# CILAB-MA/gpudrive_lab

Hardware: AMD Instinct MI355X
Metric: agent-steps/sec at 1024 worlds x 64 agents; achieved HBM GB/s on obs kernel (higher is better)
Workload: dtype f32

## Files before the change

gpudrive_lab_amd/csrc/map_obs_rank.hip:

```cpp
#include <hip/hip_runtime.h>

#include <algorithm>
#include <type_traits>

#include "engine.hpp"
#include "gd_math.hpp"
#include "rank_cand.hpp"
#include "rank_heap.hpp"

namespace gd {

namespace {

constexpr int K = GD_MAP_OBS_K;
constexpr int CAP = GD_RANK_CAP;
constexpr int NCP = GD_RANK_NCP;
constexpr int SPL = GD_RANK_SPL;
constexpr int KT = GD_RANK_KT;
constexpr int TILE = 32;
constexpr int CAP_LONG = GD_RANK_CAP_LONG;
template <int CAP_T>
struct RankGeo {
    static constexpr bool LONG = CAP_T > CAP;
    static constexpr int NG = CAP_T / 64;
    static constexpr int NMAX = CAP_T - 8;
    static constexpr int NB = CAP_T;
    static constexpr int NLIN = CAP_T * 3 / 5;
    static constexpr int TSH = LONG ? 6 : 5;
    static constexpr int RSH = LONG ? 4 : 5;
    static constexpr int KTN = LONG ? GD_RANK_KT_LONG : GD_RANK_KT;
};
constexpr int NB = RankGeo<CAP>::NB;
static_assert(K + (NCP - 1) * TILE >= CAP && K + (NCP - 1) * 64 >= CAP_LONG, "a checkpoint slot for every tile of candidates");
static_assert(CAP % 64 == 0 && NB % 128 == 0 && CAP < 2047 && CAP_LONG % 640 == 0 && CAP_LONG < 4095, "geometry; less + 1 fits 11 / 12 bits");
static_assert(SPL >= K + 31 && SPL <= CAP && KT >= CAP / 16 + 1, "every slot the finish looks up; an entry per 16 slots + the last");
constexpr int RK_FAR = 1 << 30;
constexpr int RK_TIES = 1 << 30;

__device__ __forceinline__ void wave_sync() {
    __builtin_amdgcn_fence(__ATOMIC_RELEASE, "wavefront");
    __builtin_amdgcn_wave_barrier();
    __builtin_amdgcn_fence(__ATOMIC_ACQUIRE, "wavefront");
}

__device__ __forceinline__ int wave_incl_scan(int v) {
    v += __builtin_amdgcn_update_dpp(0, v, 0x111, 0xf, 0xf, false);
    v += __builtin_amdgcn_update_dpp(0, v, 0x112, 0xf, 0xf, false);
    v += __builtin_amdgcn_update_dpp(0, v, 0x114, 0xf, 0xf, false);
    v += __builtin_amdgcn_update_dpp(0, v, 0x118, 0xf, 0xf, false);
    v += __builtin_amdgcn_update_dpp(0, v, 0x142, 0xa, 0xf, false);
    v += __builtin_amdgcn_update_dpp(0, v, 0x143, 0xc, 0xf, false);
    return v;
}

#define GD_DPP_SELF(v, ctrl, rows) __builtin_amdgcn_update_dpp((v), (v), (ctrl), (rows), 0xf, false)
__device__ __forceinline__ int wave_max(int v) {
    v = max(v, GD_DPP_SELF(v, 0x111, 0xf));
    v = max(v, GD_DPP_SELF(v, 0x112, 0xf));
    v = max(v, GD_DPP_SELF(v, 0x114, 0xf));
    v = max(v, GD_DPP_SELF(v, 0x118, 0xf));
    v = max(v, GD_DPP_SELF(v, 0x142, 0xa));
    v = max(v, GD_DPP_SELF(v, 0x143, 0xc));
    return __builtin_amdgcn_readlane(v, 63);
}
__device__ __forceinline__ float wave_max_nonneg(float f) { return __int_as_float(wave_max(__float_as_int(f))); }
__device__ __forceinline__ float wave_min_nonneg(float f) { return __int_as_float(~wave_max(~__float_as_int(f))); }
__device__ __forceinline__ int wave_sum(int v) { return __builtin_amdgcn_readlane(wave_incl_scan(v), 63); }
__device__ __forceinline__ int bits_below_lane(unsigned long long b) {
    return (int)__builtin_amdgcn_mbcnt_hi((unsigned int)(b >> 32), __builtin_amdgcn_mbcnt_lo((unsigned int)b, 0u));
}

#ifndef GD_NT_FINISH_LOAD
#define GD_NT_FINISH_LOAD 1
#endif
#ifndef GD_NT_REPLAY_LOAD
#define GD_NT_REPLAY_LOAD 1
#endif
typedef unsigned int u4v __attribute__((ext_vector_type(4)));
typedef unsigned int u2v __attribute__((ext_vector_type(2)));
template <typename T>
__device__ __forceinline__ T stream_load(const T *p) { return __builtin_nontemporal_load(p); }
template <typename T>
__device__ __forceinline__ void stream_store(T v, T *p) { __builtin_nontemporal_store(v, p); }
__device__ __forceinline__ uint4 stream_load(const uint4 *p) {
    const u4v v = __builtin_nontemporal_load(reinterpret_cast<const u4v *>(p));
    return make_uint4(v.x, v.y, v.z, v.w);
}
__device__ __forceinline__ void stream_store(uint4 v, uint4 *p) {
    u4v t; t.x = v.x; t.y = v.y; t.z = v.z; t.w = v.w;
    __builtin_nontemporal_store(t, reinterpret_cast<u4v *>(p));
}
__device__ __forceinline__ uint2 stream_load(const uint2 *p) {
    const u2v v = __builtin_nontemporal_load(reinterpret_cast<const u2v *>(p));
    return make_uint2(v.x, v.y);
}
__device__ __forceinline__ void stream_store(uint2 v, uint2 *p) {
    u2v t; t.x = v.x; t.y = v.y;
    __builtin_nontemporal_store(t, reinterpret_cast<u2v *>(p));
}

__device__ __forceinline__ int audited(const DevSim &d, int idx, int size) {
    if ((unsigned int)idx < (unsigned int)size) return idx;
    atomicAdd(&d.rk_hist[GD_RANK_AUDIT], 1);
    return idx < 0 ? 0 : size - 1;
}

__device__ __forceinline__ bool rank_lt(unsigned int a, unsigned int b, unsigned int tm = 31u) { return (a | tm) < b; }

template <int A_T>
__global__ __launch_bounds__(256) void k_knn_scan(DevSim d) {
    if (d.gate_any && *d.any_reset == 0) return;
    constexpr int HALVES = A_T / 64;
    const int w = blockIdx.x / HALVES, a0 = (blockIdx.x % HALVES) * 64;
    const int tid = threadIdx.x, wave = tid >> 6, lane = tid & 63;
    const int n = d.shape[w * 2 + 0];
    if (a0 >= n) return;
    const int a = a0 + lane;
    const bool live = a < n;
    const size_t i = (size_t)w * A_T + a;
    const size_t WA = (size_t)d.W * A_T;
    const int r0 = d.road_off[w];
    const int R = d.road_off[w + 1] - r0;

    __shared__ unsigned short s_first[NCP][64];
    __shared__ float s_thr[NCP][64];
    __shared__ int s_ncp[64];
    __shared__ unsigned int s_needy[2];
    __shared__ float4 s_hdr[64];
    __shared__ float s_bx[64], s_by[64], s_bm[64];
    __shared__ unsigned int s_hist[4][256];

    float ex = 0.f, ey = 0.f;
    if (live) { ex = d.px[i]; ey = d.py[i]; }
    unsigned long long ranked = 0ull;
    int list_base = 0;
    if (wave == 0) {
        int ncp = 0;
        float4 h0 = make_float4(0.f, 0.f, __int_as_float(0), 0.f), h1 = h0;
        if (live) { h0 = d.cp_hdr[i]; h1 = d.cp_hdr[WA + i]; }
        s_hdr[lane] = h0;
        wave_sync();
        if (live) {
            const float4 bb = d.road_bbox[w];
            const float ddx = fmaxf(fmaxf(bb.x - ex, ex - bb.z), 0.f), ddy = fmaxf(fmaxf(bb.y - ey, ey - bb.w), 0.f);
            const float far = d.p.observationRadius * 1.01f + 1.f;
            int state = 1, reason = -1;
            if (R >= K && ddx * ddx + ddy * ddy > far * far) {
                state = RK_FAR;
                d.sel_hdr[i * 2] = make_float4(ex, ey, d.qw[i], d.qz[i]);
                d.sel_hdr[i * 2 + 1] = make_float4(__int_as_float(0), __int_as_float(r0), 0.f, 0.f);
                d.cp_hdr[i] = make_float4(ex, ey, __int_as_float(0), 0.f);
            } else {
                const int n0 = __float_as_int(h0.z), n1 = __float_as_int(h1.z);
                const float m0 = n0 > 0 ? sqrtf((ex - h0.x) * (ex - h0.x) + (ey - h0.y) * (ey - h0.y)) : __builtin_inff();
                const float m1 = n1 > 0 ? sqrtf((ex - h1.x) * (ex - h1.x) + (ey - h1.y) * (ey - h1.y)) : __builtin_inff();
                int set = m1 < m0 ? 1 : 0;
                float move = set ? m1 : m0;
                int n_cp = set ? n1 : n0;
                size_t src = i;
                if (move > 6.f) {
                    float best = move;
                    int donor = -1;
                    for (int j = 0; j < 64; j++) {
                        const float4 hj = s_hdr[j];
                        const float dj = __float_as_int(hj.z) > 0 ? sqrtf((ex - hj.x) * (ex - hj.x) + (ey - hj.y) * (ey - hj.y)) : __builtin_inff();
                        if (dj < best) { best = dj; donor = j; }
                    }
                    if (donor >= 0) {
                        move = best;
                        set = 0;
                        n_cp = __float_as_int(s_hdr[donor].z);
                        src = (size_t)w * A_T + a0 + donor;
                    }
                }
                const bool eligible = R >= K && R >= d.rk_min_roads && R <= d.rk_max_roads;
                const int grp = (int)(i / 32);
                const bool bypass = eligible && d.rk_streak[grp] >= 3 && ((d.rk_hist[513] + grp) & 63) != 0;
                const float iw = d.qw[i], iz = d.qz[i];
                const float z2 = iz * iz;
                const float det = (1.f - 2.f * z2) * (1.f - 2.f * z2) + 4.f * z2 * (iw * iw);
                const float margin = 1.00001f / fminf(det, 1.f);
                if (!eligible || bypass) {
                    state = 0;
                    ncp = 0;
                    reason = bypass ? -5 : -2;
                    d.rk_fallback[i / 32] = 1;
                } else if (n_cp <= 0 || move > 6.f) {
                    ncp = -1;
                    s_bx[lane] = ex; s_by[lane] = ey; s_bm[lane] = margin;
                } else {
                    ncp = n_cp;
                    const unsigned short *cr = d.cp_road + ((size_t)set * WA + src) * NCP;
                    const float *ct = d.cp_T + ((size_t)set * WA + src) * NCP;
                    float t = 1.f;
                    unsigned int fmax = 0u;
                    for (int q = 0; q < ncp; q++) {
                        t = ct[q];
                        const float reach = sqrtf(t) * 1.0001f + move * 1.0001f + 1e-3f;
                        float thr = reach * reach * 1.0001f * margin;
                        if (!(thr >= 0.f)) thr = __builtin_inff();
                        fmax = rank_cand::running_max(fmax, cr[q]);
                        s_first[q][lane] = (unsigned short)fmax;
                        s_thr[q][lane] = thr;
                    }
                    d.rk_tl[i] = t;
                }
            }
            d.rk_n[i] = state;
            d.rk_ticket[i] = reason;
            if (state == RK_FAR) ncp = 0;
        }
        s_ncp[lane] = ncp;
        {
            const unsigned long long nd = __ballot(ncp < 0);
            if (lane == 0) { s_needy[0] = (unsigned int)nd; s_needy[1] = (unsigned int)(nd >> 32); }
        }
        if (ncp < 0) ncp = 1;
        ranked = __ballot(ncp > 0);
        if (ranked != 0ull && lane == 0) list_base = atomicAdd(&d.rk_hist[528 + (blockIdx.x & 7)], __popcll(ranked));
    }
    __syncthreads();
    {
        const unsigned long long needy = (unsigned long long)s_needy[0] | (unsigned long long)s_needy[1] << 32;
        if (needy != 0ull) {
            constexpr int BASE = (127 - 2) << 4;
            unsigned int *hist = s_hist[wave];
            int turn = 0;
            for (unsigned long long rest = needy; rest != 0ull; rest &= rest - 1ull, turn++) {
                if ((turn & 3) != wave) continue;
                const int al = __ffsll((long long)rest) - 1;
                const float bx = s_bx[al], by = s_by[al], mg = s_bm[al];
#pragma unroll
                for (int k = 0; k < 4; k++) hist[k * 64 + lane] = 0u;
                if (lane == 0) { s_first[0][al] = (unsigned short)((K / 32) * 32); s_thr[0][al] = __builtin_inff(); }
                const float ratio = exp2f(log2f(fmaxf((float)R / 256.f, 1.f)) / (float)(NCP - 2));
                float pf = 256.f, tlast = __builtin_inff();
                int pq = 256, q = 1;
                float2 nxt = lane < R ? d.road_xy[r0 + lane] : make_float2(0.f, 0.f);
                for (int rb = 0; rb < R; rb += 64) {
                    const float2 xy = nxt;
                    if (rb + 64 + lane < R) nxt = d.road_xy[r0 + rb + 64 + lane];
                    if (rb + lane < R) {
                        const float dx = xy.x - bx, dy = xy.y - by;
                        const float d2 = __builtin_fmaf(dx, dx, dy * dy);
                        atomicAdd(&hist[min(255, max(0, (int)(__float_as_uint(d2) >> 19) - BASE))], 1u);
                    }
                    if (rb + 64 == pq && q < NCP && pq < R) {
                        wave_sync();
                        const uint4 h = reinterpret_cast<const uint4 *>(hist)[lane];
                        const int own = (int)(h.x + h.y + h.z + h.w);
                        const int incl = wave_incl_scan(own), excl = incl - own;
                        int jb = 0, before = excl;
                        if (before + (int)h.x < K) { before += (int)h.x; jb = 1;
                            if (before + (int)h.y < K) { before += (int)h.y; jb = 2;
                                if (before + (int)h.z < K) { jb = 3; } } }
                        const unsigned long long cross = __ballot(excl < K && incl >= K);
                        const int Lc = __ffsll((long long)cross) - 1;
                        const int bucket = 4 * Lc + __builtin_amdgcn_readlane(jb, Lc);
                        const float T = bucket >= 255 ? __builtin_inff() : __uint_as_float((unsigned int)(bucket + 1 + BASE) << 19);
                        if (lane == 0) {
                            const float reach = sqrtf(T) * 1.0001f + 1e-3f;
                            float thr = reach * reach * 1.0001f * mg * 1.001f;
                            if (!(thr >= 0.f)) thr = __builtin_inff();
                            s_first[q][al] = (unsigned short)min(pq, 65535);
                            s_thr[q][al] = thr;
                        }
                        tlast = T;
                        q++;
                        pf *= ratio;
                        pq = max(pq + 64, ((int)pf + 63) & ~63);
                    }
                }
                if (lane == 0) {
                    s_ncp[al] = q;
                    d.rk_tl[(size_t)w * A_T + a0 + al] = tlast < 1e30f ? tlast : 1.f;
                }
            }
            __syncthreads();
        }
    }
    const int ncp = s_ncp[lane];
    if (__syncthreads_or(ncp > 0 ? 1 : 0) == 0) return;
    {
        uint2 *rows = d.rk_cp + ((size_t)w * A_T + a0) * NCP;
        for (int e = tid; e < 64 * NCP; e += 256) {
            const int ag = e / NCP, q = e - ag * NCP;
            const int n_ag = s_ncp[ag];
            if (n_ag > 0)
                rows[e] = q < n_ag ? make_uint2((unsigned int)s_first[q][ag], __float_as_uint(s_thr[q][ag]))
                                   : make_uint2(rank_cand::NO_CP, __float_as_uint(__builtin_inff()));
        }
    }
    if (wave == 0 && ranked != 0ull) {
        list_base = __builtin_amdgcn_readfirstlane(list_base);
        if (ncp > 0)
            d.rk_list[(size_t)(blockIdx.x & 7) * WA + audited(d, list_base + __popcll(ranked & ((1ull << lane) - 1ull)), (int)WA)] = (int)i;
    }
}

template <int CAP_T>
struct RankLds {
    union {
        struct {
            float ckey[CAP_T];
            unsigned short cidx[CAP_T];
        } c;
        struct {
            float skey[CAP_T];
            unsigned short spos[CAP_T];
        } s;
        unsigned short spc[CAP_T];
    };
    unsigned int cnt2[RankGeo<CAP_T>::NB / 2];
};
static_assert(sizeof(RankLds<CAP>) <= 10240 && sizeof(RankLds<CAP_LONG>) <= 20480, "sixteen / eight waves per CU");
constexpr int LSTN = (GD_MAX_ROAD_ENTITIES + GD_LIN_BLK - 1) / GD_LIN_BLK + 15;
constexpr int LSTN4 = (LSTN + 3) & ~3;
static_assert(LSTN4 <= 1024 && NCP < 64 && rank_cand::CHUNK % GD_LIN_BLK == 0 && 64 % GD_LIN_BLK == 0, "block and count share 16 bits; a block inside one chunk; whole blocks per pass");
constexpr size_t CAND_TABLES = LSTN4 * sizeof(unsigned short) + (NCP + 1) * sizeof(float);
static_assert(CAND_TABLES <= sizeof(RankLds<CAP>::cnt2) && CAND_TABLES <= sizeof(RankLds<CAP_LONG>::cnt2), "the tables fit the idle counters of both instantiations");

struct RankIn {
    int i, state, r0, R, b0, li;
    float ex, ey, iw, iz, t_last;
    unsigned int cfirst;
    float cthr;
};
template <typename T>
__device__ __forceinline__ T uniform_load(const T *p) {
    return *reinterpret_cast<const __attribute__((address_space(4))) T *>(reinterpret_cast<uintptr_t>(p));
}
template <int A_T>
__device__ __forceinline__ RankIn rank_fetch(const DevSim &d, const int *list, int li, int count, int lane) {
    RankIn in;
    in.li = li;
    in.i = li < count ? uniform_load(list + li) : 0;
    in.state = li < count ? uniform_load(d.rk_n + in.i) : 0;
    const int w = in.i / A_T;
    in.r0 = uniform_load(d.road_off + w);
    in.R = uniform_load(d.road_off + w + 1) - in.r0;
    in.ex = uniform_load(d.px + in.i); in.ey = uniform_load(d.py + in.i);
    in.iw = uniform_load(d.qw + in.i); in.iz = -uniform_load(d.qz + in.i);
    in.t_last = uniform_load(d.rk_tl + in.i);
    in.b0 = uniform_load(d.blk_off + w);
    uint2 cp = make_uint2(rank_cand::NO_CP, __float_as_uint(__builtin_inff()));
    if (in.state == 1 && lane < NCP) cp = stream_load(d.rk_cp + (size_t)in.i * NCP + (unsigned int)lane);
    in.cfirst = cp.x;
    in.cthr = __uint_as_float(cp.y);
    return in;
}

#ifdef GD_CLOCKS
struct PhaseClock {
    unsigned int prev, sum[8];
    __device__ __forceinline__ void mark(int n) {
        const unsigned int t = (unsigned int)__builtin_amdgcn_s_memtime();
        sum[n] += t - prev;
        prev = t;
    }
};
#define GD_PHASE(n) clk.mark(n)
#else
struct PhaseClock {};
#define GD_PHASE(n)
#endif
template <int A_T, int CAP_T>
__device__ __forceinline__ void rank_agent(const DevSim &d, const RankIn &in, int lane, RankLds<CAP_T> &L, PhaseClock &clk, int next_entry,
                                           int count, const int *list, RankIn &nxt) {
    using G = RankGeo<CAP_T>;
    constexpr int NB = G::NB, NLIN = G::NLIN, NMAX = G::NMAX;
    constexpr unsigned int TM = (1u << G::RSH) - 1u;
    if (__builtin_amdgcn_readfirstlane(in.state) != 1) {
        nxt = rank_fetch<A_T>(d, list, next_entry, count, lane);
        return;
    }
    auto uni = [](int v) -> int { return __builtin_amdgcn_readfirstlane(v); };
    auto unif = [](float v) -> float { return __int_as_float(__builtin_amdgcn_readfirstlane(__float_as_int(v))); };
    const int i = uni(in.i), r0 = uni(in.r0), R = uni(in.R);
    const int group = i / 32;
    constexpr int NG = G::NG;

    const float ex = unif(in.ex), ey = unif(in.ey), iw = unif(in.iw), iz = unif(in.iz);
    unsigned short *const lst = reinterpret_cast<unsigned short *>(L.cnt2);
    float *const tthr = reinterpret_cast<float *>(L.cnt2) + LSTN4 / 2;
    const unsigned int cfirst = in.cfirst;
    if (lane < NCP) tthr[lane + 1] = in.cthr;
    if (lane == 63) tthr[0] = __builtin_inff();
    const float creach = rank_cand::block_reach(in.cthr);
    const int nblk = (R + GD_LIN_BLK - 1) / GD_LIN_BLK;
    const float4 *blk = d.road_blk + uni(in.b0);
    int nsv = 0;
    constexpr int CU = 4;
#pragma clang loop unroll(disable)
    for (int b0 = 0; b0 < nblk; b0 += 64 * CU) {
        float4 c[CU];
#pragma unroll
        for (int u = 0; u < CU; u++) c[u] = blk[(unsigned int)min(b0 + u * 64 + lane, nblk - 1)];
#pragma unroll
        for (int u = 0; u < CU; u++) {
            const int bb = b0 + u * 64;
            if (bb < nblk) {
                const int b = bb + lane;
                const unsigned int base = (unsigned int)rank_cand::chunk_base_of_block(b, GD_LIN_BLK);
                const unsigned int base_lo = (unsigned int)rank_cand::chunk_base_of_block(bb, GD_LIN_BLK);
                const unsigned int base_hi = (unsigned int)rank_cand::chunk_base_of_block(min(bb + 63, nblk - 1), GD_LIN_BLK);
                const int nlo = __popcll(__ballot(cfirst <= base_lo)), nhi = __popcll(__ballot(cfirst <= base_hi));
                int cnt = nlo;
                for (int q = nlo; q < nhi; q++) cnt += (unsigned int)__builtin_amdgcn_readlane((int)cfirst, q) <= base ? 1 : 0;
                const float reach = __int_as_float(__builtin_amdgcn_ds_bpermute(((cnt - 1) & 63) << 2, __float_as_int(creach)));
                const bool sv = b < nblk && rank_cand::block_survives(b, GD_LIN_BLK, K, c[u].x, c[u].y, c[u].z, ex, ey, reach);
                const unsigned long long m = __ballot(sv);
                if (sv) lst[audited(d, nsv + bits_below_lane(m), LSTN4)] = (unsigned short)(b | cnt << 10);
                nsv += __popcll(m);
            }
        }
    }
    wave_sync();
    int nin = 0;
    {
        constexpr int BPP = 64 / GD_LIN_BLK, PB = 2;
        const int np = (nsv + BPP - 1) / BPP;
        const int sub = lane / GD_LIN_BLK, o = lane % GD_LIN_BLK;
        const float2 *rxy = d.road_xy + r0;
        struct Batch { int r[PB]; float thr[PB]; float2 xy[PB]; };
        auto issue = [&](Batch &bt, int p0) {
#pragma unroll
            for (int u = 0; u < PB; u++) {
                const int e = (p0 + u) * BPP + sub;
                const unsigned int ent = lst[min(e, LSTN4 - 1)];
                const bool on = e < nsv;
                const int r = on ? (int)(ent & 1023u) * GD_LIN_BLK + o : R;
                bt.r[u] = r;
                bt.thr[u] = tthr[on ? min((int)(ent >> 10), NCP) : 0];
                bt.xy[u] = rxy[(unsigned int)min(r, R - 1)];
            }
        };
        auto take = [&](const Batch &bt) {
#pragma unroll
            for (int u = 0; u < PB; u++) {
                const bool cand = rank_cand::is_candidate(bt.r[u], K, R, bt.xy[u].x, bt.xy[u].y, ex, ey, bt.thr[u]);
                const float key = ego_dist2(ex, ey, iw, iz, bt.xy[u].x, bt.xy[u].y);
                const unsigned long long m = __ballot(cand);
                const int pos = nin + bits_below_lane(m);
                if (cand && pos < CAP_T) {
                    L.c.cidx[pos] = (unsigned short)bt.r[u];
                    L.c.ckey[pos] = key;
                }
                nin += __popcll(m);
            }
        };
        Batch ba, bb;
        issue(ba, 0);
#pragma clang loop unroll(disable)
        for (int p0 = 0; p0 < np; p0 += 2 * PB) {
            issue(bb, p0 + PB);
            take(ba);
            if (p0 + PB >= np) break;
            issue(ba, p0 + 2 * PB);
            take(bb);
        }
    }
    wave_sync();
    nxt = rank_fetch<A_T>(d, list, next_entry, count, lane);
    {
        const int total = nin;
        if (total > NMAX) {
            if (lane == 0) {
                bool passed_on = false;
                if (!G::LONG && total <= RankGeo<CAP_LONG>::NMAX) {
                    const int slot = atomicAdd(&d.rk_hist[GD_RH_LONG], 1);
                    if (slot < d.rk_nlong) {
                        d.rk_longlist[slot] = i;
                        passed_on = true;
                    }
                }
                if (!passed_on) {
                    d.rk_n[i] = 0;
                    d.rk_ticket[i] = -3;
                    d.rk_fallback[group] = 1;
                }
            }
            return;
        }
    }
#ifdef GD_CLOCKS
    clk.sum[7] += (unsigned int)((nsv + 3) / 4) << 8;
#endif
    const int bin = 255 - min(255, (nin - K) / 5);
    int ticket = 0;
    if (lane == 0) ticket = bin << 20 | atomicAdd(&d.rk_hist[bin], 1);
    GD_PHASE(1);
    if (GD_DIAG_IS(d.rk_dbg, 1)) return;
    if (lane <= (nin - K) >> G::TSH) {
        const int road = (int)L.c.cidx[K - 1 + (lane << G::TSH)];
        d.cp_road[(size_t)i * NCP + lane] = (unsigned short)(lane ? min(65535, (road + 1 + 31) & ~31) : (K / 32) * 32);
    }
    constexpr int GQ = 5;
    static_assert(NG % GQ == 0, "whole groups");
    const float kmax = d.radius_key_max;
    int ci[NG];
    float key[NG];
    const float t_last = unif(in.t_last);
    float split = (t_last > 0.f && t_last < 1e30f) ? t_last * 1.5f : 1.f;
    int nle = 0, nlow = 0;
    float kmax_seen = 0.f, kmin_seen = __builtin_inff();
#pragma unroll
    for (int g0 = 0; g0 < NG; g0 += GQ) {
#pragma unroll
        for (int u = 0; u < GQ; u++) { ci[g0 + u] = 0; key[g0 + u] = 0.f; }
        if (g0 * 64 < nin) {
            int v[GQ];
            float kv[GQ];
#pragma unroll
            for (int u = 0; u < GQ; u++) {
                v[u] = (int)L.c.cidx[(g0 + u) * 64 + lane];
                kv[u] = L.c.ckey[(g0 + u) * 64 + lane];
            }
            static_assert(GQ == 5, "operand list");
            asm volatile("" : "+v"(v[0]), "+v"(v[1]), "+v"(v[2]), "+v"(v[3]), "+v"(v[4]), "+v"(kv[0]), "+v"(kv[1]), "+v"(kv[2]), "+v"(kv[3]), "+v"(kv[4]));
#pragma unroll
            for (int u = 0; u < GQ; u++) {
                const int g = g0 + u;
                const bool on = g * 64 + lane < nin;
                ci[g] = on ? v[u] : 0;
                key[g] = on ? kv[u] : 0.f;
                nle += ((on & (key[g] <= kmax)) ? 1 : 0) + ((on & (key[g] < split)) ? 1 << 16 : 0);
                kmax_seen = fmaxf(kmax_seen, key[g]);
                kmin_seen = fminf(kmin_seen, on ? key[g] : __builtin_inff());
            }
        }
    }
    wave_sync();
    nle = wave_sum(nle);
    kmax_seen = wave_max_nonneg(kmax_seen);
    kmin_seen = wave_min_nonneg(kmin_seen);
    nlow = nle >> 16;
    nle &= 0xffff;
    GD_PHASE(2);
    if (GD_DIAG_IS(d.rk_dbg, 2)) return;

    for (int b = lane; b < NB / 2; b += 64) L.cnt2[b] = 0u;
    wave_sync();
    const bool jumped = nlow * 4 < nin || nlow == nin;
    const float lin_lo = jumped ? kmin_seen : 0.f;
    const int nlin = jumped ? NB : NLIN;
    const float lin_scale = jumped ? (float)NB / fmaxf(kmax_seen - kmin_seen, 1e-30f) : (float)NLIN / split;
    if (jumped) split = __builtin_inff();
    const unsigned int split_bits = __float_as_uint(split);
    const float log_scale = (float)(NB - NLIN) / (float)(max(__float_as_uint(kmax_seen), split_bits + 1u) - split_bits + 1u);
    auto bucket_of = [&](float k) -> int {
        if (k < split) return min(nlin - 1, max(0, (int)((k - lin_lo) * lin_scale)));
        return NLIN + min(NB - NLIN - 1, (int)((float)(__float_as_uint(k) - split_bits) * log_scale));
    };
#pragma unroll
    for (int g = 0; g < NG; g++) {
        if (g * 64 < nin) {
            const int b = bucket_of(key[g]);
            ci[g] |= b << 16;
            if (g * 64 + lane < nin) atomicAdd(&L.cnt2[b >> 1], 1u << ((b & 1) * 16));
        }
    }
    wave_sync();
    {
        constexpr int WPB = NB / 64 / 2;
        static_assert(WPB * 128 == NB, "whole counter words per lane");
        unsigned int own[WPB];
        int sum = 0;
#pragma unroll
        for (int k = 0; k < WPB; k++) { own[k] = L.cnt2[lane * WPB + k]; sum += (int)(own[k] & 0xffffu) + (int)(own[k] >> 16); }
        int run = wave_incl_scan(sum) - sum;
#pragma unroll
        for (int k = 0; k < WPB; k++) {
            const int lo = run, hi = run + (int)(own[k] & 0xffffu);
            run = hi + (int)(own[k] >> 16);
            L.cnt2[lane * WPB + k] = (unsigned int)lo | (unsigned int)hi << 16;
        }
    }
    wave_sync();
    GD_PHASE(3);
    if (GD_DIAG_IS(d.rk_dbg, 3)) return;
#pragma unroll
    for (int g0 = 0; g0 < NG; g0 += GQ) {
        if (g0 * 64 < nin) {
            int sl[GQ];
#pragma unroll
            for (int u = 0; u < GQ; u++) {
                const int b = ci[g0 + u] >> 16, sh = (b & 1) * 16;
                const unsigned int one = (g0 + u) * 64 + lane < nin ? 1u << sh : 0u;
                sl[u] = (int)((atomicAdd(&L.cnt2[b >> 1], one) >> sh) & 0xffffu);
            }
#pragma unroll
            for (int u = 0; u < GQ; u++) {
                if ((g0 + u) * 64 + lane < nin) {
                    L.s.skey[sl[u]] = key[g0 + u];
                    L.s.spos[sl[u]] = (unsigned short)((g0 + u) * 64 + lane);
                }
            }
        }
    }
    wave_sync();
    GD_PHASE(4);
    if (GD_DIAG_IS(d.rk_dbg, 4)) return;
    const unsigned short *cur16 = reinterpret_cast<const unsigned short *>(L.cnt2);
    unsigned int eqmask = 0u;
    float *const kt_row = G::LONG ? d.rk_kt_long + (size_t)uni(in.li) * G::KTN : d.rk_kt + (size_t)i * G::KTN;
    if (lane == 0) kt_row[(nin + 15) >> 4] = kmax_seen;
    constexpr int U = 4, M = 6, STEP = 4;
    const int lim = nin;
    if (lane < 8) L.s.skey[nin + lane] = __builtin_inff();
    wave_sync();
#pragma unroll
    for (int g0 = 0; g0 < NG; g0 += U) {
        if (g0 * 64 >= nin) break;
        int s0[U], s1[U], less[U], eq[U], longest = 0;
#pragma unroll
        for (int u = 0; u < U; u++) {
            const int b = ci[g0 + u] >> 16;
            s0[u] = b ? (int)cur16[b - 1] : 0;
            s1[u] = (g0 + u) * 64 + lane < nin ? (int)cur16[b] : s0[u];
        }
#pragma unroll
        for (int u = 0; u < U; u++) {
            float mk[M];
            static_assert(M <= 8, "end markers");
#pragma unroll
            for (int k = 0; k < M; k++) mk[k] = L.s.skey[s0[u] + k];
            less[u] = s0[u];
            eq[u] = 0;
            longest = max(longest, s1[u] - s0[u]);
#pragma unroll
            for (int k = 0; k < M; k++) {
                less[u] += mk[k] < key[g0 + u] ? 1 : 0;
                eq[u] += mk[k] == key[g0 + u] ? 1 : 0;
            }
        }
        longest = wave_max(longest);
        if (GD_DIAG_IS(d.rk_dbg, 7)) longest = 0;
#ifdef GD_DIAG
        if (lane == 0 && d.rk_dbg == 9) atomicMax(&d.rk_hist[514], longest);
#endif
        for (int j = M; j < longest; j += STEP) {
            float mkk[U][STEP];
#pragma unroll
            for (int u = 0; u < U; u++)
#pragma unroll
                for (int k = 0; k < STEP; k++) mkk[u][k] = L.s.skey[min(s0[u] + j + k, lim)];
#pragma unroll
            for (int u = 0; u < U; u++)
#pragma unroll
                for (int k = 0; k < STEP; k++) {
                    less[u] += mkk[u][k] < key[g0 + u] ? 1 : 0;
                    eq[u] += mkk[u][k] == key[g0 + u] ? 1 : 0;
                }
        }
#pragma unroll
        for (int u = 0; u < U; u++) {
            const bool on = (g0 + u) * 64 + lane < nin;
            eqmask |= ((eq[u] > 1) & on) ? 1u << (g0 + u) : 0u;
            ci[g0 + u] = (ci[g0 + u] & 0xffff) | ((less[u] + 1) << (16 + G::RSH));
            const int j = (less[u] + 15) >> 4;
            if (on && (j << 4) < less[u] + eq[u]) kt_row[j] = key[g0 + u];
        }
    }
    int too_many_ties = 0;
    const bool has_tie = __ballot(eqmask != 0u) != 0ull;
    if (has_tie) {
#pragma clang loop unroll(disable)
        for (int g = 0; g * 64 < nin; g++) {
            if (__ballot((eqmask >> g) & 1u) == 0ull) continue;
            int cg = 0;
#pragma unroll
            for (int k = 0; k < NG; k++) cg = k == g ? ci[k] : cg;
            int tie = 0;
            if ((eqmask >> g) & 1u) {
                const int less_g = (int)((unsigned int)cg >> (16 + G::RSH)) - 1, p = g * 64 + lane;
                int lo = 0, hi = NB - 1;
#pragma clang loop unroll(disable)
                while (lo < hi) {
                    const int mid = (lo + hi) >> 1;
                    if ((int)cur16[mid] > less_g) hi = mid; else lo = mid + 1;
                }
                const int b = lo;
                const int first = b ? (int)cur16[b - 1] : 0, end = (int)cur16[b];
                float kg = 0.f;
                for (int m = first; m < end; m++) kg = (int)L.s.spos[m] == p ? L.s.skey[m] : kg;
                for (int m = first; m < end; m++) tie += (L.s.skey[m] == kg ? 1 : 0) & ((int)L.s.spos[m] < p ? 1 : 0);
            }
            too_many_ties |= tie > (int)TM ? 1 : 0;
#pragma unroll
            for (int k = 0; k < NG; k++) ci[k] |= k == g ? (tie & (int)TM) << 16 : 0;
        }
    }
    wave_sync();
    GD_PHASE(5);
    if (GD_DIAG_IS(d.rk_dbg, 5)) return;
    if (__ballot(too_many_ties != 0) != 0ull) {
        if (lane == 0) {
            d.rk_n[i] = 0;
            d.rk_ticket[i] = ticket | RK_TIES;
            d.rk_fallback[group] = 1;
        }
        return;
    }
    unsigned short *const E_row = G::LONG ? d.rk_E_long + (size_t)uni(in.li) * CAP_LONG : d.rk_E + (size_t)i * CAP;
    const unsigned int ulane = (unsigned int)lane;
#pragma unroll
    for (int g = 0; g < NG; g++) {
        if (g * 64 < nin) {
            if (g * 64 + lane < nin) {
                const unsigned int e = (unsigned int)ci[g] >> 16;
                stream_store((unsigned short)e, E_row + (g * 64u + ulane));
                const int slot = (int)(e >> G::RSH) - 1 + (int)(e & TM);
                if (slot < SPL) L.spc[slot] = (unsigned short)(ci[g] & 0xffff);
            }
        }
    }
    wave_sync();
    {
        static_assert(SPL == 256, "four slots per lane");
        const uint2 v = reinterpret_cast<const uint2 *>(L.spc)[lane];
        stream_store(v, reinterpret_cast<uint2 *>(d.rk_spc + (size_t)i * SPL) + ulane);
    }
    if (lane == 0) {
        d.rk_n[i] = nin | (nle << 16) | (has_tie ? 1 << 28 : 0) | (G::LONG ? 1 << 29 : 0);
        if (G::LONG) d.rk_longslot[i] = uni(in.li);
        d.rk_ticket[i] = ticket;
    }
    GD_PHASE(6);
}

template <int A_T, int CAP_T>
__global__ __launch_bounds__(64, CAP_T > CAP ? 2 : 4) void k_knn_rank(DevSim d) {
    if (d.gate_any && *d.any_reset == 0) return;
    __shared__ RankLds<CAP_T> L;
    constexpr bool LONG = RankGeo<CAP_T>::LONG;
    const int stride = LONG ? (int)gridDim.x : (int)(gridDim.x >> 3);
    const int xcd = blockIdx.x & 7;
    const int count = LONG ? min(uniform_load(d.rk_hist + GD_RH_LONG), d.rk_nlong) : uniform_load(d.rk_hist + 528 + xcd);
    const int *list = LONG ? d.rk_longlist : d.rk_list + (size_t)xcd * d.W * A_T;
    int t = LONG ? (int)blockIdx.x : (int)(blockIdx.x >> 3);
    RankIn cur = rank_fetch<A_T>(d, list, t, count, threadIdx.x);
    PhaseClock clk;
#ifdef GD_CLOCKS
    for (int k = 0; k < 8; k++) clk.sum[k] = 0u;
    clk.prev = (unsigned int)__builtin_amdgcn_s_memtime();
#endif
    for (; t < count; t += stride) {
        RankIn nxt;
        GD_PHASE(0);
        int lane_v = threadIdx.x;
        asm volatile("" : "+v"(lane_v));
        rank_agent<A_T, CAP_T>(d, cur, lane_v, L, clk, t + stride, count, list, nxt);
        wave_sync();
        cur = nxt;
    }
#ifdef GD_CLOCKS
    if (threadIdx.x == 0)
        for (int k = 0; k < 8; k++) atomicAdd(reinterpret_cast<unsigned int *>(&d.rk_hist[516 + k]), clk.sum[k] >> 8);
#endif
}

#ifndef GD_RANK_AWR
// ... 411 lines not shown
```

gpudrive_lab_amd/csrc/rank_cand.hpp:

```cpp
#pragma once

#include <cmath>

#if defined(__HIPCC__)
#define GD_RC_FN __host__ __device__ __forceinline__
#else
#define GD_RC_FN inline
#endif

namespace gd {
namespace rank_cand {

constexpr int CHUNK = 32;
constexpr unsigned int NO_CP = 0xffffffffu;

GD_RC_FN unsigned int f32_bits(float f) { return __builtin_bit_cast(unsigned int, f); }

GD_RC_FN bool road_passes(float x, float y, float ex, float ey, float thr) {
    const float dx = x - ex, dy = y - ey;
    const float d2 = __builtin_fmaf(dx, dx, dy * dy);
    return (f32_bits(d2 - thr) >> 31) != 0u;
}
GD_RC_FN bool is_candidate(int r, int K, int R, float x, float y, float ex, float ey, float thr) {
    return r < R && (r < K || road_passes(x, y, ex, ey, thr));
}

GD_RC_FN int cp_in_force(const unsigned int *first, int ncp, int base) {
    int q = -1;
    while (q + 1 < ncp && first[q + 1] <= (unsigned int)base) q++;
    return q;
}
GD_RC_FN unsigned int running_max(unsigned int run, unsigned int first) { return first > run ? first : run; }
GD_RC_FN int cp_count(const unsigned int *first_max, int n, int base) {
    int c = 0;
    for (int q = 0; q < n; q++) c += first_max[q] <= (unsigned int)base ? 1 : 0;
    return c;
}
GD_RC_FN int chunk_base_of_block(int b, int blk) { return (b * blk) & ~(CHUNK - 1); }

GD_RC_FN float block_reach(float thr) { return sqrtf(thr) * 1.00001f; }
GD_RC_FN bool block_survives(int b, int blk, int K, float cx, float cy, float rad, float ex, float ey, float reach) {
    const float dx = cx - ex, dy = cy - ey, rr = reach + rad;
    return b * blk < K || !(dx * dx + dy * dy > rr * rr * 1.00001f);
}

}
}
```

Before: 65.83 million.

## Precompute per-chunk checkpoint table in LDS and add unguarded fast candidate pass

Before scanning road blocks, the kernel builds a per-chunk table in LDS that holds the checkpoint count and reach, using an atomicMax scatter followed by a wave prefix-max. This replaces the per-block ballot and readlane loop over checkpoints. The candidate gather gets a fast path that reads packed list entries as words with bitfield extracts and skips the CAP bounds check while there is room, with a guarded tail loop handling the rest. It also drops the audited store in favour of an overflow counter. In exchange it adds LDS setup and barriers per agent and reuses the candidate-key region as scratch space.

```diff
diff --git a/gpudrive_lab_amd/csrc/map_obs_rank.hip b/gpudrive_lab_amd/csrc/map_obs_rank.hip
--- a/gpudrive_lab_amd/csrc/map_obs_rank.hip
+++ b/gpudrive_lab_amd/csrc/map_obs_rank.hip
@@ -53,6 +53,16 @@
     return v;
 }
 
+__device__ __forceinline__ int wave_incl_max_nonneg(int v) {
+    v = max(v, __builtin_amdgcn_update_dpp(0, v, 0x111, 0xf, 0xf, false));
+    v = max(v, __builtin_amdgcn_update_dpp(0, v, 0x112, 0xf, 0xf, false));
+    v = max(v, __builtin_amdgcn_update_dpp(0, v, 0x114, 0xf, 0xf, false));
+    v = max(v, __builtin_amdgcn_update_dpp(0, v, 0x118, 0xf, 0xf, false));
+    v = max(v, __builtin_amdgcn_update_dpp(0, v, 0x142, 0xa, 0xf, false));
+    v = max(v, __builtin_amdgcn_update_dpp(0, v, 0x143, 0xc, 0xf, false));
+    return v;
+}
+
 #define GD_DPP_SELF(v, ctrl, rows) __builtin_amdgcn_update_dpp((v), (v), (ctrl), (rows), 0xf, false)
 __device__ __forceinline__ int wave_max(int v) {
     v = max(v, GD_DPP_SELF(v, 0x111, 0xf));
@@ -66,6 +76,7 @@
 __device__ __forceinline__ float wave_max_nonneg(float f) { return __int_as_float(wave_max(__float_as_int(f))); }
 __device__ __forceinline__ float wave_min_nonneg(float f) { return __int_as_float(~wave_max(~__float_as_int(f))); }
 __device__ __forceinline__ int wave_sum(int v) { return __builtin_amdgcn_readlane(wave_incl_scan(v), 63); }
+__device__ __forceinline__ unsigned long long wave_ballot(bool p) { return __builtin_amdgcn_ballot_w64(p); }
 __device__ __forceinline__ int bits_below_lane(unsigned long long b) {
     return (int)__builtin_amdgcn_mbcnt_hi((unsigned int)(b >> 32), __builtin_amdgcn_mbcnt_lo((unsigned int)b, 0u));
 }
@@ -319,6 +330,8 @@
 static_assert(LSTN4 <= 1024 && NCP < 64 && rank_cand::CHUNK % GD_LIN_BLK == 0 && 64 % GD_LIN_BLK == 0, "block and count share 16 bits; a block inside one chunk; whole blocks per pass");
 constexpr size_t CAND_TABLES = LSTN4 * sizeof(unsigned short) + (NCP + 1) * sizeof(float);
 static_assert(CAND_TABLES <= sizeof(RankLds<CAP>::cnt2) && CAND_TABLES <= sizeof(RankLds<CAP_LONG>::cnt2), "the tables fit the idle counters of both instantiations");
+constexpr int CP_EPL = ((GD_MAX_ROAD_ENTITIES + rank_cand::CHUNK - 1) / rank_cand::CHUNK + 63) / 64;
+static_assert(64 * CP_EPL * (sizeof(unsigned int) + sizeof(uint2)) <= sizeof(float) * CAP, "the chunk table fits the candidate keys of both instantiations");
 
 struct RankIn {
     int i, state, r0, R, b0, li;
@@ -388,30 +401,61 @@
     if (lane == 63) tthr[0] = __builtin_inff();
     const float creach = rank_cand::block_reach(in.cthr);
     const int nblk = (R + GD_LIN_BLK - 1) / GD_LIN_BLK;
+    const int nch = rank_cand::chunks_of(R), epl = (nch + 63) >> 6;
+    unsigned int *const tmax = reinterpret_cast<unsigned int *>(L.c.ckey);
+    uint2 *const tcp = reinterpret_cast<uint2 *>(L.c.ckey + 64 * CP_EPL);
+#pragma unroll
+    for (int u = 0; u < CP_EPL; u++)
+        if (u < epl) tmax[u * 64 + lane] = 0u;
+    wave_sync();
+    if (lane < NCP && rank_cand::cp_table_takes(cfirst, nch)) atomicMax(&tmax[rank_cand::cp_table_chunk(cfirst)], rank_cand::cp_table_entry(lane));
+    wave_sync();
+    {
+        int own[CP_EPL], run = 0;
+#pragma unroll
+        for (int u = 0; u < CP_EPL; u++) own[u] = u < epl ? (int)tmax[lane * epl + u] : 0;
+#pragma unroll
+        for (int u = 0; u < CP_EPL; u++) { run = max(run, own[u]); own[u] = run; }
+        const int before = __builtin_amdgcn_ds_bpermute(((lane - 1) & 63) << 2, wave_incl_max_nonneg(run));
+#pragma unroll
+        for (int u = 0; u < CP_EPL; u++)
+            if (u < epl) {
+                const int cnt = lane ? max(own[u], before) : own[u];
+                const int reach = __builtin_amdgcn_ds_bpermute(((cnt - 1) & 63) << 2, __float_as_int(creach));
+                tcp[lane * epl + u] = make_uint2((unsigned int)cnt, (unsigned int)reach);
+            }
+    }
+    wave_sync();
     const float4 *blk = d.road_blk + uni(in.b0);
     int nsv = 0;
     constexpr int CU = 4;
 #pragma clang loop unroll(disable)
     for (int b0 = 0; b0 < nblk; b0 += 64 * CU) {
         float4 c[CU];
-#pragma unroll
-        for (int u = 0; u < CU; u++) c[u] = blk[(unsigned int)min(b0 + u * 64 + lane, nblk - 1)];
+        uint2 cp[CU];
+#pragma unroll
+        for (int u = 0; u < CU; u++) {
+            const int bc = min(b0 + u * 64 + lane, nblk - 1);
+            c[u] = blk[(unsigned int)bc];
+            cp[u] = tcp[rank_cand::chunk_base_of_block(bc, GD_LIN_BLK) / rank_cand::CHUNK];
+        }
+        static_assert(CU == 4, "operand list");
+        asm volatile("" : "+v"(c[0].x), "+v"(c[0].y), "+v"(c[0].z), "+v"(c[1].x), "+v"(c[1].y), "+v"(c[1].z), "+v"(c[2].x), "+v"(c[2].y), "+v"(c[2].z),
+                     "+v"(c[3].x), "+v"(c[3].y), "+v"(c[3].z));
 #pragma unroll
         for (int u = 0; u < CU; u++) {
             const int bb = b0 + u * 64;
             if (bb < nblk) {
                 const int b = bb + lane;
-                const unsigned int base = (unsigned int)rank_cand::chunk_base_of_block(b, GD_LIN_BLK);
-                const unsigned int base_lo = (unsigned int)rank_cand::chunk_base_of_block(bb, GD_LIN_BLK);
-                const unsigned int base_hi = (unsigned int)rank_cand::chunk_base_of_block(min(bb + 63, nblk - 1), GD_LIN_BLK);
-                const int nlo = __popcll(__ballot(cfirst <= base_lo)), nhi = __popcll(__ballot(cfirst <= base_hi));
-                int cnt = nlo;
-                for (int q = nlo; q < nhi; q++) cnt += (unsigned int)__builtin_amdgcn_readlane((int)cfirst, q) <= base ? 1 : 0;
-                const float reach = __int_as_float(__builtin_amdgcn_ds_bpermute(((cnt - 1) & 63) << 2, __float_as_int(creach)));
-                const bool sv = b < nblk && rank_cand::block_survives(b, GD_LIN_BLK, K, c[u].x, c[u].y, c[u].z, ex, ey, reach);
-                const unsigned long long m = __ballot(sv);
-                if (sv) lst[audited(d, nsv + bits_below_lane(m), LSTN4)] = (unsigned short)(b | cnt << 10);
-                nsv += __popcll(m);
+                const bool sv = b < nblk && rank_cand::block_survives(b, GD_LIN_BLK, K, c[u].x, c[u].y, c[u].z, ex, ey, __uint_as_float(cp[u].y));
+                const unsigned long long m = wave_ballot(sv);
+                const int upto = nsv + __popcll(m);
+                if (upto <= LSTN4) {
+                    if (sv) lst[nsv + bits_below_lane(m)] = (unsigned short)((unsigned int)b | cp[u].x << 10);
+                    nsv = upto;
+                } else if (lane == 0) {
+                    atomicAdd(&d.rk_hist[GD_RANK_AUDIT], 1);
+                }
             }
         }
     }
@@ -419,45 +463,85 @@
     int nin = 0;
     {
         constexpr int BPP = 64 / GD_LIN_BLK, PB = 2;
-        const int np = (nsv + BPP - 1) / BPP;
+        const int np = (nsv + BPP - 1) / BPP, nfast = np - 1;
         const int sub = lane / GD_LIN_BLK, o = lane % GD_LIN_BLK;
         const float2 *rxy = d.road_xy + r0;
-        struct Batch { int r[PB]; float thr[PB]; float2 xy[PB]; };
-        auto issue = [&](Batch &bt, int p0) {
-#pragma unroll
-            for (int u = 0; u < PB; u++) {
-                const int e = (p0 + u) * BPP + sub;
-                const unsigned int ent = lst[min(e, LSTN4 - 1)];
-                const bool on = e < nsv;
-                const int r = on ? (int)(ent & 1023u) * GD_LIN_BLK + o : R;
-                bt.r[u] = r;
-                bt.thr[u] = tthr[on ? min((int)(ent >> 10), NCP) : 0];
-                bt.xy[u] = rxy[(unsigned int)min(r, R - 1)];
-            }
+        auto store = [&](bool cand, int r, float key, unsigned long long m, bool guard) {
+            const int pos = nin + bits_below_lane(m);
+            if (cand && (!guard || pos < CAP_T)) {
+                L.c.cidx[pos] = (unsigned short)r;
+                L.c.ckey[pos] = key;
+            }
+            nin += __popcll(m);
         };
-        auto take = [&](const Batch &bt) {
-#pragma unroll
-            for (int u = 0; u < PB; u++) {
-                const bool cand = rank_cand::is_candidate(bt.r[u], K, R, bt.xy[u].x, bt.xy[u].y, ex, ey, bt.thr[u]);
-                const float key = ego_dist2(ex, ey, iw, iz, bt.xy[u].x, bt.xy[u].y);
-                const unsigned long long m = __ballot(cand);
-                const int pos = nin + bits_below_lane(m);
-                if (cand && pos < CAP_T) {
-                    L.c.cidx[pos] = (unsigned short)bt.r[u];
-                    L.c.ckey[pos] = key;
-                }
-                nin += __popcll(m);
-            }
-        };
-        Batch ba, bb;
-        issue(ba, 0);
+        int p = 0;
+        if (nfast >= 2 * PB) {
+            const unsigned int *lsub = reinterpret_cast<const unsigned int *>(L.cnt2) + sub / 2;
+            const unsigned int sh = (unsigned int)(sub & 1) * 16u;
+            const unsigned int o8 = (unsigned int)o * (unsigned int)sizeof(float2);
+            static_assert(BPP == 4, "two words per pass");
+            struct Ents { unsigned int e[PB]; };
+            struct Batch { unsigned int off[PB]; float thr[PB]; float2 xy[PB]; };
+            auto entries = [&](Ents &en, int p0) {
+#pragma unroll
+                for (int u = 0; u < PB; u++) en.e[u] = lsub[min(p0 + u, nfast - 1) * (BPP / 2)];
+            };
+            auto issue = [&](Batch &bt, const Ents &en) {
+#pragma unroll
+                for (int u = 0; u < PB; u++) {
+                    bt.off[u] = __builtin_amdgcn_ubfe(en.e[u], sh, 10u) * (unsigned int)(GD_LIN_BLK * sizeof(float2)) + o8;
+                    bt.thr[u] = tthr[__builtin_amdgcn_ubfe(en.e[u], sh + 10u, 6u)];
+                    bt.xy[u] = *reinterpret_cast<const float2 *>(reinterpret_cast<const char *>(rxy) + bt.off[u]);
+                }
+            };
+            auto take = [&](const Batch &bt) {
+#pragma unroll
+                for (int u = 0; u < PB; u++) {
+                    const int r = (int)(bt.off[u] / (unsigned int)sizeof(float2));
+                    __builtin_assume(r >= 0 && r < R);
+                    const bool cand = rank_cand::is_candidate(r, K, R, bt.xy[u].x, bt.xy[u].y, ex, ey, bt.thr[u]);
+                    store(cand, r, ego_dist2(ex, ey, iw, iz, bt.xy[u].x, bt.xy[u].y), wave_ballot(cand), false);
+                }
+            };
+            Ents ea, eb;
+            Batch ba, bb;
+            entries(ea, 0);
+            entries(eb, PB);
+            issue(ba, ea);
 #pragma clang loop unroll(disable)
-        for (int p0 = 0; p0 < np; p0 += 2 * PB) {
-            issue(bb, p0 + PB);
-            take(ba);
-            if (p0 + PB >= np) break;
-            issue(ba, p0 + 2 * PB);
-            take(bb);
+            for (; p + 2 * PB <= nfast && nin + 2 * PB * 64 <= CAP_T; p += 2 * PB) {
+                issue(bb, eb);
+                entries(ea, p + 2 * PB);
+                take(ba);
+                issue(ba, ea);
+                entries(eb, p + 3 * PB);
+                take(bb);
+            }
+        }
+#pragma clang loop unroll(disable)
+        for (; p < np; p += 2 * PB) {
+            int r[2 * PB];
+            float thr[2 * PB];
+            float2 xy[2 * PB];
+#pragma unroll
+            for (int u = 0; u < 2 * PB; u++) {
+                r[u] = R; thr[u] = 0.f; xy[u] = make_float2(0.f, 0.f);
+                if (p + u < np) {
+                    const int e = (p + u) * BPP + sub;
+                    const unsigned int ent = lst[min(e, LSTN4 - 1)];
+                    const bool on = e < nsv;
+                    r[u] = on ? (int)(ent & 1023u) * GD_LIN_BLK + o : R;
+                    thr[u] = tthr[on ? min((int)(ent >> 10), NCP) : 0];
+                    xy[u] = rxy[(unsigned int)min(r[u], R - 1)];
+                }
+            }
+#pragma unroll
+            for (int u = 0; u < 2 * PB; u++) {
+                if (p + u < np) {
+                    const bool cand = rank_cand::is_candidate(r[u], K, R, xy[u].x, xy[u].y, ex, ey, thr[u]);
+                    store(cand, r[u], ego_dist2(ex, ey, iw, iz, xy[u].x, xy[u].y), wave_ballot(cand), true);
+                }
+            }
         }
     }
     wave_sync();
diff --git a/gpudrive_lab_amd/csrc/rank_cand.hpp b/gpudrive_lab_amd/csrc/rank_cand.hpp
--- a/gpudrive_lab_amd/csrc/rank_cand.hpp
+++ b/gpudrive_lab_amd/csrc/rank_cand.hpp
@@ -38,6 +38,22 @@
 }
 GD_RC_FN int chunk_base_of_block(int b, int blk) { return (b * blk) & ~(CHUNK - 1); }
 
+GD_RC_FN int chunks_of(int R) { return (R + CHUNK - 1) / CHUNK; }
+GD_RC_FN unsigned int cp_table_chunk(unsigned int first_max) { return first_max / CHUNK + (first_max % CHUNK ? 1u : 0u); }
+GD_RC_FN bool cp_table_takes(unsigned int first_max, int nchunks) {
+    return first_max != NO_CP && cp_table_chunk(first_max) < (unsigned int)nchunks;
+}
+GD_RC_FN unsigned int cp_table_entry(int q) { return (unsigned int)q + 1u; }
+GD_RC_FN void cp_table(unsigned int *tab, int nchunks, const unsigned int *first_max, int n) {
+    for (int c = 0; c < nchunks; c++) tab[c] = 0u;
+    for (int q = 0; q < n; q++)
+        if (cp_table_takes(first_max[q], nchunks)) {
+            unsigned int &e = tab[cp_table_chunk(first_max[q])];
+            e = cp_table_entry(q) > e ? cp_table_entry(q) : e;
+        }
+    for (int c = 1; c < nchunks; c++) tab[c] = tab[c - 1] > tab[c] ? tab[c - 1] : tab[c];
+}
+
 GD_RC_FN float block_reach(float thr) { return sqrtf(thr) * 1.00001f; }
 GD_RC_FN bool block_survives(int b, int blk, int K, float cx, float cy, float rad, float ex, float ey, float reach) {
     const float dx = cx - ex, dy = cy - ey, rr = reach + rad;
```

Result: faster. 67.51 million, median of 6 (+2.6%).
